# ChristianSteger/HORAYZON

Measured on AMD Instinct MI355X. Metric: grid_cells_per_s (horizon_gridded, 360 azimuths, 3601^2 SRTM-like tile), higher is better.
Workload: dtype f32

## Files before the change

### horayzon_amd/csrc/hz_common.h

```cpp
#pragma once
#include <stdint.h>
#include <hip/hip_runtime.h>

#define HZ_BLOB_MAGIC 0x485a4c42u
#define HZ_BLOB_VERSION 10u
#define HZ_WAVE 64

struct BlobHeader {
    uint32_t magic, version;
    int32_t d0, d1;
    int32_t n_quads, n_tin, n_prims, n_nodes;
    int32_t height, n_top;
    float center[3];
    float pad;
    float lo[3], hi[3];
    uint32_t reserved0[2];
    uint64_t off_verts, off_nodes, off_prims, total_bytes;
    uint64_t off_anc;
    int32_t anc_levels;
    int32_t n_prim_slots;
    uint32_t flags;
    uint32_t n_flipped;
    uint64_t off_bad;
    int32_t bad_nb;
// ... 223 lines not shown
typedef int hz_int2 __attribute__((ext_vector_type(2)));

__device__ __forceinline__ float hz_fma_mix_lo(uint32_t h2, float a, float b) {
    return __builtin_fmaf((float)__builtin_bit_cast(hz_half2, h2).x, a, b);
}
__device__ __forceinline__ float hz_fma_mix_hi(uint32_t h2, float a, float b) {
    return __builtin_fmaf((float)__builtin_bit_cast(hz_half2, h2).y, a, b);
}

__device__ __forceinline__ void hz_node_hits(const NodeRay &n, const RayBox &r, float tfar, const uint4 &q,
                                             bool &h0, bool &h1, bool &h2, bool &h3) {
    const uint32_t px0 = __builtin_amdgcn_perm(HZ_HALF_MAGIC, q.x, r.sel_x), px1 = __builtin_amdgcn_perm(HZ_HALF_MAGIC, q.x, r.sel_x + HZ_SEL_PAIR1);
    const uint32_t py0 = __builtin_amdgcn_perm(HZ_HALF_MAGIC, q.y, r.sel_y), py1 = __builtin_amdgcn_perm(HZ_HALF_MAGIC, q.y, r.sel_y + HZ_SEL_PAIR1);
    const uint32_t pz0 = __builtin_amdgcn_perm(HZ_HALF_MAGIC, q.z, r.sel_z), pz1 = __builtin_amdgcn_perm(HZ_HALF_MAGIC, q.z, r.sel_z + HZ_SEL_PAIR1);
    const uint32_t pz2 = __builtin_amdgcn_perm(HZ_HALF_MAGIC, q.w, r.sel_z), pz3 = __builtin_amdgcn_perm(HZ_HALF_MAGIC, q.w, r.sel_z + HZ_SEL_PAIR1);
    const float nx0 = hz_fma_mix_lo(px0, n.ax, n.bx), fx0 = hz_fma_mix_hi(px0, n.ax, n.bx);
    const float nx1 = hz_fma_mix_lo(px1, n.ax, n.bx), fx1 = hz_fma_mix_hi(px1, n.ax, n.bx);
    const float ny0 = hz_fma_mix_lo(py0, n.ay, n.by), fy0 = hz_fma_mix_hi(py0, n.ay, n.by);
    const float ny1 = hz_fma_mix_lo(py1, n.ay, n.by), fy1 = hz_fma_mix_hi(py1, n.ay, n.by);
    const float cx0 = __builtin_fmaxf(nx0, 0.0f), cx1 = __builtin_fmaxf(nx1, 0.0f);
    const float gx0 = __builtin_fminf(fx0, tfar), gx1 = __builtin_fminf(fx1, tfar);
#define HZ_CHILD(pz, nx, fx, ny, fy, out) do { \
        const float nz_ = hz_fma_mix_lo(pz, n.az, n.bz), fz_ = hz_fma_mix_hi(pz, n.az, n.bz); \
        const float tmin_ = __builtin_fmaxf(__builtin_fmaxf(nx, ny), nz_); \
        const float tmax_ = __builtin_fminf(__builtin_fminf(fx, fy), fz_); \
        out = tmin_ <= tmax_ * 1.000001f; } while (0)
    HZ_CHILD(pz0, cx0, gx0, ny0, fy0, h0);
    HZ_CHILD(pz1, cx1, gx1, ny0, fy0, h1);
    HZ_CHILD(pz2, cx0, gx0, ny1, fy1, h2);
    HZ_CHILD(pz3, cx1, gx1, ny1, fy1, h3);
#undef HZ_CHILD
}

__device__ __forceinline__ void hz_node_hit_masks(const NodeRay &n, const RayBox &r, float tfar, const uint4 &q,
                                                  int &m0, int &m1, int &m2, int &m3) {
    const uint32_t px0 = __builtin_amdgcn_perm(HZ_HALF_MAGIC, q.x, r.sel_x), px1 = __builtin_amdgcn_perm(HZ_HALF_MAGIC, q.x, r.sel_x + HZ_SEL_PAIR1);
    const uint32_t py0 = __builtin_amdgcn_perm(HZ_HALF_MAGIC, q.y, r.sel_y), py1 = __builtin_amdgcn_perm(HZ_HALF_MAGIC, q.y, r.sel_y + HZ_SEL_PAIR1);
    const uint32_t pz0 = __builtin_amdgcn_perm(HZ_HALF_MAGIC, q.z, r.sel_z), pz1 = __builtin_amdgcn_perm(HZ_HALF_MAGIC, q.z, r.sel_z + HZ_SEL_PAIR1);
    const uint32_t pz2 = __builtin_amdgcn_perm(HZ_HALF_MAGIC, q.w, r.sel_z), pz3 = __builtin_amdgcn_perm(HZ_HALF_MAGIC, q.w, r.sel_z + HZ_SEL_PAIR1);
    const float nx0 = hz_fma_mix_lo(px0, n.ax, n.bx), fx0 = hz_fma_mix_hi(px0, n.ax, n.bx);
    const float nx1 = hz_fma_mix_lo(px1, n.ax, n.bx), fx1 = hz_fma_mix_hi(px1, n.ax, n.bx);
    const float ny0 = hz_fma_mix_lo(py0, n.ay, n.by), fy0 = hz_fma_mix_hi(py0, n.ay, n.by);
    const float ny1 = hz_fma_mix_lo(py1, n.ay, n.by), fy1 = hz_fma_mix_hi(py1, n.ay, n.by);
    const float cx0 = __builtin_fmaxf(nx0, 0.0f), cx1 = __builtin_fmaxf(nx1, 0.0f);
    const float gx0 = __builtin_fminf(fx0, tfar), gx1 = __builtin_fminf(fx1, tfar);
#define HZ_CHILD_M(pz, nx, fx, ny, fy, out) do { \
        const float nz_ = hz_fma_mix_lo(pz, n.az, n.bz), fz_ = hz_fma_mix_hi(pz, n.az, n.bz); \
        const float tmin_ = __builtin_fmaxf(__builtin_fmaxf(nx, ny), nz_); \
        const float tmax_ = __builtin_fminf(__builtin_fminf(fx, fy), fz_); \
        out = __float_as_int(__builtin_fmaf(tmax_, -1.000001f, tmin_)) >> 31; \
        asm volatile("" : "+v"(out));      \
        } while (0)
    HZ_CHILD_M(pz0, cx0, gx0, ny0, fy0, m0);
    HZ_CHILD_M(pz1, cx1, gx1, ny0, fy0, m1);
    HZ_CHILD_M(pz2, cx0, gx0, ny1, fy1, m2);
    HZ_CHILD_M(pz3, cx1, gx1, ny1, fy1, m3);
#undef HZ_CHILD_M
}

__device__ __forceinline__ void hz_load_node(const Node *n, float4 &n0, uint4 &n1) {
    asm volatile("global_load_dwordx4 %0, %2, off\n\t"
                 "global_load_dwordx4 %1, %2, off offset:16\n\t"
                 "s_waitcnt vmcnt(0)"
                 : "=&v"(n0), "=&v"(n1)
                 : "v"(n)
                 : "memory");
}

__device__ __forceinline__ void hz_load_node_lds(const float4 *q, float4 &n0, uint4 &n1) {
    const unsigned addr = (unsigned)(size_t)reinterpret_cast<const __attribute__((address_space(3))) char *>(
        (const __attribute__((address_space(3))) float4 *)q);
    asm volatile("ds_read_b128 %0, %2\n\t"
                 "ds_read_b128 %1, %2 offset:16\n\t"
                 "s_waitcnt lgkmcnt(0)"
                 : "=&v"(n0), "=&v"(n1)
                 : "v"(addr)
                 : "memory");
}

__device__ __forceinline__ void hz_load_prim(const Prim *q, float4 &q0, float4 &q1, float4 &q2) {
    asm volatile("global_load_dwordx4 %0, %3, off\n\t"
                 "global_load_dwordx4 %1, %3, off offset:16\n\t"
                 "global_load_dwordx4 %2, %3, off offset:32\n\t"
                 "s_waitcnt vmcnt(0)"
                 : "=&v"(q0), "=&v"(q1), "=&v"(q2)
                 : "v"(q)
                 : "memory");
}

struct TravCounters { unsigned nodes, tris, w_nodes, w_leaves;
};
#endif

#if defined(__HIPCC__)
__host__ __device__
#endif
inline int hz_n_leave(int regroup, int n_entry, int rule, int round) {
    const int cap = rule ? 64 : regroup, share = rule ? regroup : 64;
    const int rel = (share * n_entry + round) >> 6;
    const int cut = cap < rel ? cap : rel;
    return cut > 1 ? cut : 1;
}

#ifdef __HIPCC__
struct LendCounters { unsigned lent, unhelped; };
struct TravState { int node, sp, pf, pm, lq0, lq1; };

__device__ __forceinline__ void hz_trav_reset(TravState &t) {
    t.node = 0; t.sp = 0; t.pf = 0; t.pm = 0; t.lq0 = HZ_EMPTY; t.lq1 = HZ_EMPTY;
}

__device__ __forceinline__ int hz_entry_pack(int pf, int pm) {
    return (int)((unsigned)pf | (((unsigned)pm >> 1) & 3u) | (((unsigned)pm & 8u) << 27));
}
__device__ __forceinline__ void hz_entry_unpack(int e, int &pf, int &pm) {
    pm = (int)((((unsigned)e & 3u) << 1) | (((unsigned)e >> 27) & 8u));
    pf = (int)((unsigned)e & 0xbffffffcu);
}

#define HZ_WAVE_TICK(c, lane_) do { const unsigned long long m_ = __ballot(1); if ((lane_) == __ffsll((long long)m_) - 1) (c)++; } while (0)

template <int TPB, bool COUNT, int QLEN = 2, bool NODELET = false, bool LEVELSTACK = true, bool LEND = false>
__device__ __forceinline__ int hz_trace(const Node *__restrict__ nodes, const Prim *__restrict__ prims,
                                        const float4 *top, int ntop, int *stack, int tid,
                                        float ox, float oy, float oz, float dx, float dy, float dz, float tfar,
                                        float tfar_box, const RayBox &rb, TravState &t, int regroup, int leaf_bias,
                                        TravCounters &cnt, int stack_cap, bool &overflow, LendCounters *lcnt = nullptr,
                                        int regroup_rule = 0) {
    const int lane = tid & 63;
    int node = t.node, sp = t.sp, pf = t.pf, pm = t.pm, lq0 = t.lq0, lq1 = t.lq1;
    const int n_entry = __popcll(__ballot(1));
#define HZ_POP() do { \
        if (LEVELSTACK) { \
            if (pm == 0) { const bool ne = sp > 0; sp = ne ? sp - 1 : 0; const int pv = stack[sp * TPB + tid]; \
                           hz_entry_unpack(ne ? pv : 0, pf, pm); } \
            const int slot_ = __builtin_ctz((unsigned)pm | 16u); \
            node = (pm != 0) ? pf + slot_ : HZ_EMPTY; pm &= pm - 1; \
        } else { \
            node = HZ_STACK_AT(sa + (unsigned)(TPB * 4)); sa -= (unsigned)(TPB * 4); \
        } } while (0)
typedef __attribute__((address_space(3))) int hz_lds_int;
#define HZ_STACK_AT(addr) (*reinterpret_cast<hz_lds_int *>((size_t)(addr)))
#define HZ_SAVE() do { if (!LEVELSTACK) sp = (int)(sa - sa0) / (TPB * 4) + 1; \
                       t.node = node; t.sp = sp; t.pf = pf; t.pm = pm; t.lq0 = lq0; t.lq1 = lq1; } while (0)
    const unsigned sa0 = (unsigned)(size_t)reinterpret_cast<hz_lds_int *>(
                             (__attribute__((address_space(3))) char *)reinterpret_cast<char *>(stack)) + (unsigned)tid * 4u;
    unsigned sa = sa0 + (unsigned)(sp - 1) * (unsigned)(TPB * 4);
    const unsigned sa_cap = sa0 + (unsigned)(stack_cap - 5) * (unsigned)(TPB * 4);
    if (!LEVELSTACK) HZ_STACK_AT(sa0) = HZ_EMPTY;
    unsigned sa_hi = 0u;
    const int n_leave = hz_n_leave(regroup, n_entry, regroup_rule & 1, regroup_rule >> 1);
    bool can_node, can_leaf;
    unsigned long long m_node, m_leaf;
    int n_all;
    auto top_of_iteration = [&]() __attribute__((always_inline)) {
        if (LEVELSTACK) {
            if (node < 0 && lq0 >= 0) { lq0 = node; HZ_POP(); }
            if (node < 0 && lq1 >= 0) { lq1 = node; HZ_POP(); }
        } else {
            hz_int2 t10;
            asm volatile("ds_read2st64_b32 %0, %1 offset1:%2\n\ts_waitcnt lgkmcnt(0)" : "=v"(t10) : "v"(sa), "n"(TPB / 64) : "memory");
            int t0 = t10.y;
            const int t1 = t10.x;
#define HZ_SELM(m, x, y) (((m) & (x)) | (~(m) & (y)))
            int m1 = (node & ~lq0) >> 31;
            asm volatile("" : "+v"(m1));
            lq0 = HZ_SELM(m1, node, lq0); node = HZ_SELM(m1, t0, node); t0 = HZ_SELM(m1, t1, t0); sa -= (unsigned)m1 & (unsigned)(TPB * 4);
            int m2 = (node & ~lq1) >> 31;
            asm volatile("" : "+v"(m2));
            lq1 = HZ_SELM(m2, node, lq1); node = HZ_SELM(m2, t0, node); sa -= (unsigned)m2 & (unsigned)(TPB * 4);
#undef HZ_SELM
        }
        can_node = HZ_IS_NODE(node);
        can_leaf = lq0 < 0;
        m_node = __ballot(can_node); m_leaf = __ballot(can_leaf);
        n_all = __popcll(m_node | m_leaf);
    };
    top_of_iteration();
    while (n_all >= n_leave) {
        const int n_node = __popcll(m_node);
        const int n_leaf = __popcll(m_leaf);
        if (n_node * 16 >= n_leaf * leaf_bias) {
            if (can_node) {
                float4 n0; uint4 n1;
                if (NODELET && node < ntop) hz_load_node_lds(top + 2 * node, n0, n1);
                else hz_load_node(nodes + node, n0, n1);
                if (COUNT) { cnt.nodes++; HZ_WAVE_TICK(cnt.w_nodes, lane); }
                const NodeRay nr = hz_node_ray(rb, n0.x, n0.y, n0.z);
                const int first = __float_as_int(n0.w);
                if (LEVELSTACK) {
                    bool h0, h1, h2, h3;
                    hz_node_hits(nr, rb, tfar_box, n1, h0, h1, h2, h3);
                    const int h = (h0 ? 1 : 0) | (h1 ? 2 : 0) | (h2 ? 4 : 0) | (h3 ? 8 : 0);
                    if (h != 0) {
                        if (pm != 0) { stack[sp * TPB + tid] = hz_entry_pack(pf, pm); sp++; }
                        pf = first; pm = h;
                    }
                    HZ_POP();
                } else {
                    int m0, m1, m2, m3;
                    hz_node_hit_masks(nr, rb, tfar_box, n1, m0, m1, m2, m3);
                    sa_hi = max(sa_hi, sa);
                    sa = min(sa, sa_cap);
                    const unsigned S = (unsigned)(TPB * 4);
                    const int pv = HZ_STACK_AT(sa + S);
                    const unsigned a0 = (unsigned)m0 & S, a1 = (unsigned)m1 & S, a2 = (unsigned)m2 & S, a3 = (unsigned)m3 & S;
                    const unsigned o32 = a3 | a2, o321 = o32 | a1, o3210 = o321 | a0;
#define HZ_SEL(m, x, y) (((m) & (x)) | (~(m) & (y)))
                    int next = HZ_SEL(m3, first + 3, pv);
                    HZ_STACK_AT(sa + 2u * S) = next; sa += a2 & a3;   next = HZ_SEL(m2, first + 2, next);
                    HZ_STACK_AT(sa + 2u * S) = next; sa += a1 & o32;  next = HZ_SEL(m1, first + 1, next);
                    HZ_STACK_AT(sa + 2u * S) = next; sa += a0 & o321; next = HZ_SEL(m0, first, next);
#undef HZ_SEL
                    node = next; sa = sa + o3210 - S;
                }
            }
        } else {
            if (LEND && !LEVELSTACK) {
                static_assert(HZ_EMPTY > 1, "the idle word must be neither a queued link (negative) nor HZ_EMPTY");
                int p_w = 0, lf;
                float rox, roy, roz, rdx, rdy, rdz;
#define HZ_DPP_SEL(d, x) "v_cndmask_b32_dpp %[" d "], %[" x "], %[" x "], vcc quad_perm:[1,0,3,2] row_mask:0xf bank_mask:0xf bound_ctrl:1\n\t"
                asm volatile("s_mov_b64 vcc, %[m]\n\t"
                             "v_cndmask_b32_e32 %[lf], 1, %[lq1], vcc\n\t"
                             HZ_DPP_SEL("rox", "ox") HZ_DPP_SEL("roy", "oy") HZ_DPP_SEL("roz", "oz")
                             HZ_DPP_SEL("rdx", "dx") HZ_DPP_SEL("rdy", "dy") HZ_DPP_SEL("rdz", "dz")
                             "v_mov_b32_dpp %[pw], %[lf] quad_perm:[1,0,3,2] row_mask:0xf bank_mask:0xf\n\t"
                             "v_cndmask_b32_e32 %[lf], %[pw], %[lq0], vcc"
                             : [pw] "+&v"(p_w), [lf] "=&v"(lf), [rox] "=&v"(rox), [roy] "=&v"(roy), [roz] "=&v"(roz),
                               [rdx] "=&v"(rdx), [rdy] "=&v"(rdy), [rdz] "=&v"(rdz)
                             : [m] "s"(m_leaf), [lq0] "v"(lq0), [lq1] "v"(lq1), [ox] "v"(ox), [oy] "v"(oy), [oz] "v"(oz),
                               [dx] "v"(dx), [dy] "v"(dy), [dz] "v"(dz)
                             : "vcc");
#undef HZ_DPP_SEL
// ... 84 lines not shown
```

### horayzon_amd/csrc/hz_horizon.hip

```cpp
#include "hz_search.h"
#include <vector>

namespace hz {

#ifndef HZ_TPB
#define HZ_TPB 256
#endif
#define HZ_WPB (HZ_TPB / 64)
#ifndef HZ_QLEN
#define HZ_QLEN 2
#endif

struct HorizonParams {
    SceneView sv;
    Tables tb;
    const float *vec_norm, *vec_north;
    const uint8_t *mask;
    float *hori;
    int offset_0, offset_1, dim_in_1;
    int row_begin, row_end;
    TileMap tm;
    float dist, hori_fill, ray_org_elev;
    float dist_box, neg_tau;
    int top_nodes, regroup, stack_bytes, leaf_bias, stage_bytes, hit_cache, stack_cap;
    int pre_bytes;
    const unsigned short *near_idx;
    const float *near_r;
    float *scratch_row;
    int verify_near;
    unsigned verify_mask;
    unsigned long long *counters;
    const int *tile_list;
    int n_list;
// ... 20 lines not shown
#ifndef HZ_WG_PER_CU
#define HZ_WG_PER_CU 5
#endif
__global__ __launch_bounds__(HZ_TPB, (COUNT ? 4 : HZ_WG_PER_CU) * (4 / HZ_WPB)) void k_horizon(HorizonParams p_arg) {
    typedef const __attribute__((address_space(4))) HorizonParams *hz_kparams;
    hz_kparams pk = (hz_kparams)__builtin_amdgcn_kernarg_segment_ptr();
#if defined(__HIP_DEVICE_COMPILE__)
#define HZ_LOAD_PARAMS(dst) dst = *pk
#else
#define HZ_LOAD_PARAMS(dst) dst = p_arg
#endif
    HorizonParams p;
    HZ_LOAD_PARAMS(p);
    extern __shared__ __attribute__((aligned(16))) unsigned char smem[];
    int *stack = reinterpret_cast<int *>(smem + p.pre_bytes);
    const float4 *top = reinterpret_cast<const float4 *>(smem + p.pre_bytes + p.stack_bytes);
    const int tid = threadIdx.x;
    const int ntop = p.top_nodes;
    if (NODELET && ntop > 0) {
        float4 *dst = reinterpret_cast<float4 *>(smem + p.pre_bytes + p.stack_bytes);
        const float4 *src = reinterpret_cast<const float4 *>(p.sv.nodes);
        for (int i = tid; i < ntop * 2; i += HZ_TPB) dst[i] = src[i];
        __syncthreads();
    }

    const int wave = __builtin_amdgcn_readfirstlane(tid >> 6);
    const int xcc_own = (int)(__builtin_amdgcn_s_getreg((3 << 11) | 20) & 7u);
    int xcc_off = 0;
    int left_on = 1;
  for (;;) {
    asm volatile("" : "+s"(pk));
    HZ_LOAD_PARAMS(p);
    int tid_b = tid;
    asm volatile("" : "+v"(tid_b));
    const int lane = tid_b & 63;
#define HZ_KEEP(x) asm volatile("" : "+s"(x))
    HZ_KEEP(p.leaf_bias); HZ_KEEP(p.regroup); HZ_KEEP(p.neg_tau); HZ_KEEP(p.sv.cx); HZ_KEEP(p.sv.cy); HZ_KEEP(p.sv.cz);
    HZ_KEEP(p.near_idx); HZ_KEEP(p.near_r);
    if (FLAT && LEFT) { HZ_KEEP(p.sv.nodes); HZ_KEEP(p.sv.prims); }
#undef HZ_KEEP
    int ti = 0, tj = 0;
    int blk = (int)blockIdx.x * HZ_WPB + wave;
    unsigned rec0 = 0u, rec_n = 0u;
    if (LEFT) {
        blk = -1;
        const unsigned groups = (p.left_in_ctl[1] + 63u) / 64u;
        if (p.tile_list) {
            const int b = (int)blockIdx.x * HZ_WPB + wave;
            const int g = b < p.n_list ? p.tile_list[b] : -1;
            if (g >= 0 && (unsigned)g < groups) { blk = g; rec0 = (unsigned)g * 64u; rec_n = min(64u, p.left_in_ctl[1] - (unsigned)g * 64u); }
        } else
        while (xcc_off < 8) {
            const unsigned x = (unsigned)((xcc_own + xcc_off) & 7);
            unsigned q = 0u;
            if (lane == 0) q = atomicAdd(&p.left_in_ctl[8 + x], 1u);
            q = (unsigned)__builtin_amdgcn_readfirstlane((int)q);
            const unsigned g = (((q >> 5) * 8u + x) << 5) | (q & 31u);
            if (g < groups) { blk = (int)g; rec0 = g * 64u; rec_n = min(64u, p.left_in_ctl[1] - g * 64u); break; }
            xcc_off++;
        }
        if (blk < 0) break;
    } else if (p.persist) {
        blk = -1;
        while (xcc_off < 8) {
            const int x = (xcc_own + xcc_off) & 7;
            int q = 0;
            if (lane == 0) q = (int)atomicAdd(&p.queue[x], 1u);
            q = __builtin_amdgcn_readfirstlane(q);
            if (q < p.tm.per_xcd * 4) { blk = (((q >> 2) * 8 + x) << 2) | (q & 3); break; }
            xcc_off++;
        }
        if (blk < 0) break;
    } else if (p.tile_list) blk = (blk < p.n_list) ? p.tile_list[blk] : -1;
// ... 1 lines not shown
        const int b = (int)blockIdx.x, x = b & 7, t = b >> 3, per = 4 / HZ_WPB;
        blk = (((t / per) * 8 + x) * 4) + (t % per) * HZ_WPB + wave;
    }
    blk = __builtin_amdgcn_readfirstlane(blk);
    bool has_tile = blk >= 0 && (LEFT || hz_tile_of_block(p.tm, blk >> 2, &ti, &tj));
    int i = p.row_begin + ti * 16 + ((blk >> 1) & 1) * 8 + (lane >> 3);
    int j = tj * 16 + (blk & 1) * 8 + (lane & 7);
    const unsigned *rec = nullptr;
    if (LEFT) {
        has_tile = (unsigned)lane < rec_n;
        if (has_tile) {
            rec = p.left_rec + ((size_t)p.left_in_base + (size_t)p.left_perm[rec0 + (unsigned)lane]) * HZ_LEFT_WORDS;
            const unsigned c0 = rec[0];
            has_tile = c0 != 0xffffffffu;
            const unsigned di = c0 / (unsigned)p.dim_in_1;
            i = p.row_begin + (int)di; j = (int)(c0 - di * (unsigned)p.dim_in_1);
        }
    }
    const bool in_dom = has_tile && (i < p.row_end) && (j < p.dim_in_1);

    const Tables &t = p.tb;
    const unsigned long long t_start = COUNT ? (unsigned long long)wall_clock64() : 0ull;
    const size_t cell = in_dom ? ((size_t)i * p.dim_in_1 + j) : 0;
    bool done = !in_dom;
    const unsigned cert = in_dom ? (unsigned)(i - p.row_begin) * (unsigned)p.dim_in_1 + (unsigned)j : 0u;
    const bool to_scratch = COUNT && p.scratch_row != nullptr;
    float *const hori0 = to_scratch ? p.scratch_row : p.hori + (size_t)p.row_begin * p.dim_in_1 * (size_t)t.azim_num;
    const unsigned cell_stride = to_scratch ? 0u : 1u;
    Sink out;
    out.hori = COUNT ? hori0 + (size_t)(cert * cell_stride) * (size_t)t.azim_num : hori0 + (size_t)cert * (size_t)t.azim_num;
    out.dist = nullptr; out.dist_hit = 0.0f;
    out.stage = reinterpret_cast<float *>(smem) + tid_b;
    out.stride = HZ_TPB;
    float ox = 0, oy = 0, oz = 0;
    float r01 = 0, r02 = 0, r11 = 0, r12 = 0, r21 = 0, r22 = 0;
    const bool masked = in_dom && p.mask[cell] != 1;
    {
        unsigned long long m = __ballot(masked);
        while (m) {
            const int src = __ffsll((long long)m) - 1;
            m &= m - 1;
            float *row = COUNT ? hori0 + (size_t)((unsigned)__shfl((int)cert, src) * cell_stride) * (size_t)t.azim_num
                               : hori0 + (size_t)__shfl((int)cert, src) * (size_t)t.azim_num;
            for (int k = lane; k < t.azim_num; k += 64) row[k] = p.hori_fill;
        }
    }
    if (in_dom) {
        if (masked) {
            done = true;
        } else {
            const float norm_x = p.vec_norm[3 * cell], norm_y = p.vec_norm[3 * cell + 1], norm_z = p.vec_norm[3 * cell + 2];
            const float north_x = p.vec_north[3 * cell], north_y = p.vec_north[3 * cell + 1], north_z = p.vec_north[3 * cell + 2];
            const float *v = p.sv.verts + 3 * ((size_t)(i + p.offset_0) * p.sv.d1 + (size_t)(j + p.offset_1));
            ox = v[0] + norm_x * p.ray_org_elev;
            oy = v[1] + norm_y * p.ray_org_elev;
            oz = v[2] + norm_z * p.ray_org_elev;
            r01 = north_x; r02 = norm_x;
            r11 = north_y; r12 = norm_y;
            r21 = north_z; r22 = norm_z;
        }
    }
#define HZ_OC(ocx, ocy, ocz) float ocx, ocy, ocz; { float ax_ = ox, ay_ = oy, az_ = oz; \
        asm volatile("" : "+v"(ax_), "+v"(ay_), "+v"(az_)); \
        ocx = ax_ - p.sv.cx; ocy = ay_ - p.sv.cy; ocz = az_ - p.sv.cz; }
    const float tfar = p.dist;

    Search s;
    s.k = 0; s.phase = PH_NEWAZ; s.ind = 0; s.prev = 0; s.pazim = 0; s.count = 0;
    s.lim_up = 0; s.lim_low = 0; s.elev_samp = 0; s.ev = 0;
    unsigned rays = 0, guards = 0, w_adv = 0;
    unsigned refill_hist = 0;
    TravCounters tc; tc.nodes = 0; tc.tris = 0; tc.w_nodes = 0; tc.w_leaves = 0;
    LendCounters lc; lc.lent = 0; lc.unhelped = 0;
    const unsigned cells_cnt = (in_dom && !done && !LEFT) ? 1u : 0u;
    bool ray_active = false, last_hit = false;
    float dx = 0, dy = 0, dz = 1;
    RayBox rb = hz_raybox(0, 0, 0, 0, 0, 1);
    TravState ts; hz_trav_reset(ts);
    int cache = 0;
    bool second = false;
    bool overflow = false;
    unsigned shortened = 0;
    unsigned w_verified = 0, w_violations = 0;
    bool verifying = false, first_result = false, want_v = false;
    float tn = 0.0f;
    bool had_guard = false;
    if (LEFT && !done) {
        s.k = (int)rec[1]; s.phase = (int)(rec[2] & 0xffu); s.ind = (int)rec[3]; s.prev = (int)rec[4]; s.pazim = (int)rec[5]; s.count = (int)rec[6];
        s.lim_up = __uint_as_float(rec[7]); s.lim_low = __uint_as_float(rec[8]); s.elev_samp = __uint_as_float(rec[9]); s.ev = __uint_as_float(rec[10]);
        cache = (int)rec[11];
        last_hit = (rec[2] & 0x100u) != 0u;
        had_guard = (rec[2] & 0x400u) != 0u;
        if (STAGE) { out.stage[0] = __uint_as_float(rec[12]); out.stage[out.stride] = __uint_as_float(rec[13]); out.stage[2 * out.stride] = __uint_as_float(rec[14]); }
        if (rec[2] & 0x200u) {
            const float ec = t.elev_cos[s.ind], es = t.elev_sin[s.ind];
            const float rx = ec * t.azim_sin[s.k], ry = ec * t.azim_cos[s.k], rz = es;
            const float r00 = r11 * r22 - r21 * r12, r10 = r21 * r02 - r01 * r22, r20 = r01 * r12 - r11 * r02;
            dx = (r00 * rx + r01 * ry) + r02 * rz;
            dy = (r10 * rx + r11 * ry) + r12 * rz;
            dz = (r20 * rx + r21 * ry) + r22 * rz;
            HZ_OC(ocx, ocy, ocz)
            rb = hz_raybox(ocx + p.neg_tau * dx, ocy + p.neg_tau * dy, ocz + p.neg_tau * dz, dx, dy, dz);
            hz_trav_reset(ts);
            ray_active = true;
        }
    }

    int left_min = (COUNT || !left_on || __popcll(__ballot(!done)) <= p.left_min + 8) ? 0 : p.left_min;
    while (__ballot(!done) != 0ull) {
        if (!COUNT && left_min > 0 && __popcll(__ballot(!done)) <= left_min) {
            const unsigned long long um = __ballot(!done);
            if (um != 0ull && !(!LEVELSTACK && __ballot(overflow) != 0ull)) {
                const unsigned n = (unsigned)__popcll(um);
                unsigned *const out_rec = p.left_rec + (size_t)p.left_out_base * HZ_LEFT_WORDS;
                unsigned base = 0u;
                if (lane == 0) base = atomicAdd(&p.left_out_ctl[0], n);
                base = (unsigned)__builtin_amdgcn_readfirstlane((int)base);
                if (base + n > p.left_out_cap) {
                    left_on = 0; left_min = 0;
                    if (base + (unsigned)lane < p.left_out_cap) out_rec[(size_t)(base + (unsigned)lane) * HZ_LEFT_WORDS] = 0xffffffffu;
                } else {
                    if (lane == 0) atomicAdd(&p.counters[LEFT ? HZ_CNT_LEFT_AGAIN : HZ_CNT_LEFT_CELLS], (unsigned long long)n);
                    if (!done) {
                        const unsigned rank = (unsigned)__builtin_amdgcn_mbcnt_hi((unsigned)(um >> 32), __builtin_amdgcn_mbcnt_lo((unsigned)um, 0u));
                        const unsigned flags = (unsigned)s.phase | (last_hit ? 0x100u : 0u) | (ray_active ? 0x200u : 0u) | ((guards != 0u || had_guard) ? 0x400u : 0u);
                        hz_left_write(out_rec + (size_t)(base + rank) * HZ_LEFT_WORDS, cert, (unsigned)s.k, flags,
                                      (unsigned)s.ind, (unsigned)s.prev, (unsigned)s.pazim, (unsigned)s.count, s.lim_up, s.lim_low, s.elev_samp, s.ev, (unsigned)cache,
                                      STAGE ? out.stage[0] : 0.0f, STAGE ? out.stage[out.stride] : 0.0f, STAGE ? out.stage[2 * out.stride] : 0.0f);
                        done = true;
                    }
                }
            }
        }

        if (__ballot(!done) == 0ull) break;
        const int n_refill = COUNT ? __popcll(__ballot(!done && !ray_active)) : 0;
        if (COUNT && n_refill > 0 && lane == ((n_refill - 1) >> 3)) refill_hist++;
        if (!done && !ray_active) {
            if (COUNT) HZ_WAVE_TICK(w_adv, lane);
            unsigned cert_r = cert;
            asm volatile("" : "+v"(cert_r));
            out.hori = COUNT ? hori0 + (size_t)(cert_r * cell_stride) * (size_t)t.azim_num : hori0 + (size_t)cert_r * (size_t)t.azim_num;
#define HZ_RAY_SETUP(GO) \
                const float rx = ec * asn, ry = ec * acs, rz = es; \
                float nx_ = r01, ny_ = r11, nz_ = r21;         \
                asm volatile("" : "+v"(nx_), "+v"(ny_), "+v"(nz_)); \
                const float r00 = ny_ * r22 - nz_ * r12;       \
                const float r10 = nz_ * r02 - nx_ * r22; \
                const float r20 = nx_ * r12 - ny_ * r02; \
                dx = (r00 * rx + r01 * ry) + r02 * rz; \
                dy = (r10 * rx + r11 * ry) + r12 * rz; \
                dz = (r20 * rx + r21 * ry) + r22 * rz; \
                    tn = (s.ind >= near_i) ? near_rad : p.neg_tau;     \
                if (COUNT && (GO) && tn > 0.0f) shortened++; \
                if (COUNT) want_v = (GO) && p.verify_near && tn > 0.0f && (((rays + cert) & p.verify_mask) == 0u); \
                HZ_OC(ocx, ocy, ocz) \
                rb = hz_raybox(ocx + tn * dx, ocy + tn * dy, ocz + tn * dz, dx, dy, dz); \
                hz_trav_reset(ts); \
                 \
                second = p.hit_cache && (cache != 0) && (s.ind <= s.pazim) && (s.k > 0); \
                if (second) { \
                    ts.node = cache; \
                     \
                    if (!LEVELSTACK) { ts.sp = 1; stack[HZ_TPB + tid] = 0; second = false; } \
                }
            if (FLAT) {
                float ec = 0.0f, es = 0.0f, asn = 0.0f, acs = 0.0f, near_rad = 0.0f;
                int near_i = 0x7fffffff;
                const bool go = advance_guess_flat<STAGE>(s, last_hit, t, out, guards,
                    [&](int kc) {
                        asn = t.azim_sin[kc]; acs = t.azim_cos[kc];
                        if (p.near_idx != nullptr) {
                            near_i = (int)p.near_idx[(size_t)cert_r * (size_t)t.azim_num + kc];
                            near_rad = p.near_r[cert_r];
                        }
                    },
                    [&](int ind) { ec = t.elev_cos[ind]; es = t.elev_sin[ind]; });
                HZ_RAY_SETUP(go)
                ray_active = go;
                done = !go;
                rays += go ? 1u : 0u;
            } else
            if (advance<ALG, STAGE>(s, last_hit, t, out, guards)) {
                const float ec = t.elev_cos[s.ind], es = t.elev_sin[s.ind];
                const float asn = t.azim_sin[s.k], acs = t.azim_cos[s.k];
                int near_i = 0x7fffffff;
                float near_rad = 0.0f;
                if (p.near_idx != nullptr) {
                    near_i = (int)p.near_idx[(size_t)cert_r * (size_t)t.azim_num + s.k];
                    near_rad = p.near_r[cert_r];
                }
                HZ_RAY_SETUP(true)
                ray_active = true;
                rays++;
            } else {
                done = true;
            }
#undef HZ_RAY_SETUP
        }
        bool start_v = false, viol = false;
        if (COUNT && n_refill > 0) {
            const int n_enter = __popcll(__ballot(ray_active));
            if (n_enter > 0 && lane == 8 + ((n_enter - 1) >> 3)) refill_hist++;
        }
        if (ray_active) {
            int r;
            r = hz_trace<HZ_TPB, COUNT, HZ_QLEN, NODELET, LEVELSTACK, LEND>(p.sv.nodes, p.sv.prims, top, ntop, stack, tid, ox, oy, oz,
                                                 dx, dy, dz, tfar, p.dist_box, rb, ts, p.regroup & 0xff, p.leaf_bias, tc, p.stack_cap, overflow, &lc, p.regroup >> 8);
            if (r == 0 && second) {
                second = false; hz_trav_reset(ts);
            } else if (COUNT && want_v && r != 2) {
                want_v = false; verifying = true; first_result = (r == 1); start_v = true;
                HZ_OC(ocx, ocy, ocz)
                rb = hz_raybox(ocx + p.neg_tau * dx, ocy + p.neg_tau * dy, ocz + p.neg_tau * dz, dx, dy, dz);
                hz_trav_reset(ts);
            } else if (r != 2) {
                if (COUNT && verifying) { viol = ((r == 1) != first_result); verifying = false; }
                ray_active = false; last_hit = (r == 1);
                if (r == 1) cache = p.sv.anc[HZ_LEAF_ID(ts.lq0)];
            }
        }
        if (COUNT) {
            w_verified += (unsigned)__popcll(__ballot(start_v));
            w_violations += (unsigned)__popcll(__ballot(viol));
        }
    }
    unsigned long long r = rays, g = guards, nc = tc.nodes, tcn = tc.tris, cc = cells_cnt;
    unsigned long long wn = tc.w_nodes, wl = tc.w_leaves, wa = w_adv;
    unsigned long long ln = lc.lent, un = lc.unhelped;
    for (int off = 32; off > 0; off >>= 1) {
        r += __shfl_xor(r, off); g += __shfl_xor(g, off); cc += __shfl_xor(cc, off);
        if (COUNT) {
            nc += __shfl_xor(nc, off); tcn += __shfl_xor(tcn, off);
            wn += __shfl_xor(wn, off); wl += __shfl_xor(wl, off); wa += __shfl_xor(wa, off);
            if (LEND) { ln += __shfl_xor(ln, off); un += __shfl_xor(un, off); }
        }
    }
    const bool wave_overflowed = !LEVELSTACK && __ballot(overflow) != 0ull;
    if (wave_overflowed) {
        if (lane == 0) {
            const unsigned long long slot = atomicAdd(&p.counters[LEFT ? HZ_CNT_LEFT_OVERFLOW : HZ_CNT_OVERFLOW], 1ull);
            if (slot < (unsigned long long)HZ_REDO_CAP) p.redo_list[(LEFT ? HZ_REDO_CAP : 0) + (int)slot] = blk;
        }
    } else {
    const int guard_cells = __popcll(__ballot(guards != 0u && !(LEFT && had_guard)));
    if (lane == 0) {
        if (r) atomicAdd(&p.counters[HZ_CNT_RAYS], r);
        if (g) { atomicAdd(&p.counters[HZ_CNT_GUARDS], g); atomicAdd(&p.counters[HZ_CNT_GUARD_CELLS], (unsigned long long)guard_cells); }
        if (cc) atomicAdd(&p.counters[HZ_CNT_CELLS], cc);
        if (COUNT) {
            atomicAdd(&p.counters[HZ_CNT_NODES], nc); atomicAdd(&p.counters[HZ_CNT_TRIS], tcn);
            atomicAdd(&p.counters[HZ_CNT_WAVE_NODE], wn); atomicAdd(&p.counters[HZ_CNT_WAVE_LEAF], wl); atomicAdd(&p.counters[HZ_CNT_WAVE_REFILL], wa);
            if (LEND) { atomicAdd(&p.counters[HZ_CNT_LENT], ln); atomicAdd(&p.counters[HZ_CNT_UNHELPED], un); }
        }
    }
    if (COUNT && lane < 16 && refill_hist != 0u) atomicAdd(&p.counters[HZ_CNT_REFILL + lane], (unsigned long long)refill_hist);
    if (COUNT) {
        if (lane == 0) {
            const unsigned xcc = __builtin_amdgcn_s_getreg((3 << 11) | 20) & 7u;
            atomicMax(&p.counters[HZ_CNT_XCD_END + xcc], (unsigned long long)wall_clock64());
            atomicMax(&p.counters[HZ_CNT_START], ~t_start);
        }
    }
    if (COUNT) {
        unsigned long long sh = shortened;
        for (int off = 32; off > 0; off >>= 1) sh += __shfl_xor(sh, off);
        if (lane == 0) {
            if (sh) atomicAdd(&p.counters[HZ_CNT_SHORTENED], sh);
            if (w_violations) atomicAdd(&p.counters[HZ_CNT_VIOLATIONS], (unsigned long long)w_violations);
            if (w_verified) atomicAdd(&p.counters[HZ_CNT_VERIFIED], (unsigned long long)w_verified);
        }
    }
    }
    if (!p.persist) break;
  }
}

std::atomic<int> g_leaf_lend{1};
std::atomic<int> g_flat_refill{1};
std::atomic<int> g_regroup_rule{1};
std::atomic<int> g_regroup_round{HZ_REGROUP_ROUND};

static long long resident_workgroups(const void *func, size_t lds) {
    struct Key { const void *f; size_t lds; int dev; long long n; };
    static std::mutex mu;
    static std::vector<Key> cache;
    int dev = 0;
    if (hipGetDevice(&dev) != hipSuccess) { (void)hipGetLastError(); return 0; }
    std::lock_guard<std::mutex> lock(mu);
    for (const Key &k : cache) if (k.f == func && k.lds == lds && k.dev == dev) return k.n;
    int per_cu = 0;
    hipDeviceProp_t prop;
    long long n = 0;
    if (hipOccupancyMaxActiveBlocksPerMultiprocessor(&per_cu, func, HZ_TPB, lds) == hipSuccess && per_cu > 0 &&
        hipGetDeviceProperties(&prop, dev) == hipSuccess && prop.multiProcessorCount > 0)
        n = (long long)per_cu * prop.multiProcessorCount;
    else (void)hipGetLastError();
    cache.push_back(Key{func, lds, dev, n});
    return n;
}

template <int ALG, bool COUNT, bool STAGE, bool NODELET, bool LEVELSTACK, bool LEND = false, bool FLAT = false>
static int launch_one(const HorizonParams &p_in, int grid, size_t lds, int persist_grid, hipStream_t st) {
    const void *func = reinterpret_cast<const void *>(k_horizon<ALG, COUNT, STAGE, NODELET, LEVELSTACK, false, LEND, FLAT>);
    HZ_HIP(hipFuncSetAttribute(func, hipFuncAttributeMaxDynamicSharedMemorySize, (int)lds));
    HorizonParams p = p_in;
    if (p.persist) {
        const long long resident = persist_grid > 0 ? (long long)persist_grid : resident_workgroups(func, lds);
// ... 512 lines not shown
```

### horayzon_amd/csrc/hz_search.h

```cpp
#pragma once
#include "hz_internal.h"

namespace hz {

enum { ALG_DISCRETE = 0, ALG_BINARY = 1, ALG_GUESS = 2 };
enum { PH_NEWAZ = 0, PH_BIN = 1, PH_UP = 2, PH_DOWN = 3, PH_EMIT = 4 };

struct Tables {
    const float *azim_sin, *azim_cos, *elev_ang, *elev_sin, *elev_cos;
    const int *mid_idx;
    int azim_num, elev_num;
    float hori_acc, low, up;
    double step;
};

struct Search {
    int k, phase, ind, prev, pazim, count;
    float lim_up, lim_low, elev_samp;
    float ev;
};

__device__ __forceinline__ int ind_of(const Tables &t, float elev_samp) {
    return (int)__builtin_roundf((float)((double)(elev_samp - t.low) / t.step));
}
// ... 85 lines not shown
            }
            if (guard) guards++;
            if (ALG == ALG_DISCRETE) {
                s.ev = half_sum(t.elev_ang[s.prev], t.elev_ang[s.ind]); s.phase = PH_EMIT;
                s.pazim = s.prev;
                continue;
            }
            if (s.count > 1) {
                s.ind = mid_index(t, s.prev, s.ind, &s.ev);
                s.pazim = s.ind; s.phase = PH_EMIT;
                continue;
            }
            s.ind = min(s.pazim + 5, top);
            s.prev = s.ind;
            s.ind = max(s.ind - 10, 0);
            s.phase = PH_DOWN;
            return true;
        }
        {
            const bool guard = (!hit) && (s.ind == 0);
            if (!hit && !guard) {
                s.prev = s.ind;
                s.ind = max(s.ind - 10, 0);
                return true;
            }
            if (guard) guards++;
            s.ind = mid_index(t, s.prev, s.ind, &s.ev);
            s.pazim = s.ind; s.phase = PH_EMIT;
            continue;
        }
    }
}

#define HZ_HIDE(m) asm volatile("" : "+v"(m))
#define HZ_BSEL(m, x, y) (((m) & (x)) | (~(m) & (y)))
template <bool STAGE, class FK, class FI>
__device__ __forceinline__ bool advance_guess_flat(Search &s, bool hit, const Tables &t, Sink &out, unsigned &guards,
                                                   FK &&issue_k, FI &&issue_ind) {
    const int top = t.elev_num - 1;
    int m_flat = (int)((unsigned)s.phase << 30) >> 31;
    HZ_HIDE(m_flat);
    if (__ballot(m_flat == 0) != 0ull) {
        if (m_flat == 0) (void)advance<ALG_GUESS, STAGE>(s, hit, t, out, guards);
    }
    int m_down = (int)((unsigned)s.phase << 31) >> 31;
    int m_hit = hit ? -1 : 0;
    int m_end = (s.ind == (top & ~m_down)) ? -1 : 0;
    int m_many = (1 - s.count) >> 31;
    HZ_HIDE(m_down); HZ_HIDE(m_hit); HZ_HIDE(m_end); HZ_HIDE(m_many);
    const int m_fwd = (m_hit ^ m_down) & m_flat;
    const int m_step = m_fwd & ~m_end;
    const int m_turn = m_flat & ~(m_step | m_down | m_many);
    const int m_fin = m_flat & ~(m_step | m_turn);
    guards += (unsigned)(m_fwd & m_end & 1);
    const int st_ind = min(max(s.ind + 10 - (20 & m_down), 0), top);
    const int tu_prev = min(s.pazim + 5, top), tu_ind = max(tu_prev - 10, 0);
    const int lo = min(s.prev, s.ind), hi = max(s.prev, s.ind);
    const int2 pair = reinterpret_cast<const int2 *>(t.mid_idx)[min(max(lo, 0), top)];
    int m_gen = (hi - lo != 10) ? m_fin : 0;
    HZ_HIDE(m_gen);
    const int k_new = s.k - m_fin;
    issue_k(min(k_new, t.azim_num - 1));
    int mid = pair.x, evb = pair.y;
    if (__ballot(m_gen != 0) != 0ull) {
        if (m_gen != 0) {
            mid = ind_of(t, half_sum(t.elev_ang[s.prev], t.elev_ang[s.ind]));
            evb = __float_as_int(t.elev_ang[mid]);
        }
    }
    const int fi_prev = max(mid - 5, 0), fi_ind = min(fi_prev + 10, top);
    const int ind_new = HZ_BSEL(m_step, st_ind, HZ_BSEL(m_turn, tu_ind, HZ_BSEL(m_fin, fi_ind, s.ind)));
    issue_ind(ind_new);
    const int k_emit = s.k;
    s.prev = HZ_BSEL(m_step, s.ind, HZ_BSEL(m_turn, tu_prev, HZ_BSEL(m_fin, fi_prev, s.prev)));
    s.ind = ind_new;
    s.count = HZ_BSEL(m_fin, 1, s.count + (m_step & ~m_down & 1));
    s.phase += m_turn & 1;
    s.phase -= m_fin & m_down & 1;
    s.pazim = HZ_BSEL(m_fin, mid, s.pazim);
    s.ev = __int_as_float(HZ_BSEL(m_fin, evb, __float_as_int(s.ev)));
    s.k = k_new;
    if (m_fin != 0) emit<STAGE>(out, t, k_emit, __int_as_float(evb));
    return s.k < t.azim_num;
}
#undef HZ_BSEL
#undef HZ_HIDE

}
```

Measured before the change: 10.93 million.

## Add lean FLAT path with slim search state and absolute LDS stack address

For the FLAT kernel variant, the search state shrinks to SearchLean: the bisection limits move into LDS staging slots and the unused ev/elev_samp fields are dropped. The traversal stack pointer is now kept as an absolute LDS byte address, and the regroup parameters are pre-packed into one scalar. The box test takes tfar as an SGPR operand through inline asm, and the sel_x1/sel_y1 selectors are hoisted out of the loop. The aim is to lower VGPR pressure and per-iteration integer work to raise occupancy, at the cost of extra LDS traffic and more complicated suspend/resume record handling.

```diff
diff --git a/horayzon_amd/csrc/hz_common.h b/horayzon_amd/csrc/hz_common.h
--- a/horayzon_amd/csrc/hz_common.h
+++ b/horayzon_amd/csrc/hz_common.h
@@ -279,10 +279,16 @@
 #undef HZ_CHILD
 }
 
-__device__ __forceinline__ void hz_node_hit_masks(const NodeRay &n, const RayBox &r, float tfar, const uint4 &q,
-                                                  int &m0, int &m1, int &m2, int &m3) {
-    const uint32_t px0 = __builtin_amdgcn_perm(HZ_HALF_MAGIC, q.x, r.sel_x), px1 = __builtin_amdgcn_perm(HZ_HALF_MAGIC, q.x, r.sel_x + HZ_SEL_PAIR1);
-    const uint32_t py0 = __builtin_amdgcn_perm(HZ_HALF_MAGIC, q.y, r.sel_y), py1 = __builtin_amdgcn_perm(HZ_HALF_MAGIC, q.y, r.sel_y + HZ_SEL_PAIR1);
+__device__ __forceinline__ float hz_min_uniform(float a, float uniform_b) {
+    float r;
+    asm("v_min_f32_e32 %0, %2, %1" : "=v"(r) : "v"(a), "s"(uniform_b));
+    return r;
+}
+template <bool LEAN>
+__device__ __forceinline__ void hz_node_hit_masks_t(const NodeRay &n, const RayBox &r, uint32_t sel_x1, uint32_t sel_y1, float tfar, const uint4 &q,
+                                                    int &m0, int &m1, int &m2, int &m3) {
+    const uint32_t px0 = __builtin_amdgcn_perm(HZ_HALF_MAGIC, q.x, r.sel_x), px1 = __builtin_amdgcn_perm(HZ_HALF_MAGIC, q.x, sel_x1);
+    const uint32_t py0 = __builtin_amdgcn_perm(HZ_HALF_MAGIC, q.y, r.sel_y), py1 = __builtin_amdgcn_perm(HZ_HALF_MAGIC, q.y, sel_y1);
     const uint32_t pz0 = __builtin_amdgcn_perm(HZ_HALF_MAGIC, q.z, r.sel_z), pz1 = __builtin_amdgcn_perm(HZ_HALF_MAGIC, q.z, r.sel_z + HZ_SEL_PAIR1);
     const uint32_t pz2 = __builtin_amdgcn_perm(HZ_HALF_MAGIC, q.w, r.sel_z), pz3 = __builtin_amdgcn_perm(HZ_HALF_MAGIC, q.w, r.sel_z + HZ_SEL_PAIR1);
     const float nx0 = hz_fma_mix_lo(px0, n.ax, n.bx), fx0 = hz_fma_mix_hi(px0, n.ax, n.bx);
@@ -290,7 +296,7 @@
     const float ny0 = hz_fma_mix_lo(py0, n.ay, n.by), fy0 = hz_fma_mix_hi(py0, n.ay, n.by);
     const float ny1 = hz_fma_mix_lo(py1, n.ay, n.by), fy1 = hz_fma_mix_hi(py1, n.ay, n.by);
     const float cx0 = __builtin_fmaxf(nx0, 0.0f), cx1 = __builtin_fmaxf(nx1, 0.0f);
-    const float gx0 = __builtin_fminf(fx0, tfar), gx1 = __builtin_fminf(fx1, tfar);
+    const float gx0 = LEAN ? hz_min_uniform(fx0, tfar) : __builtin_fminf(fx0, tfar), gx1 = LEAN ? hz_min_uniform(fx1, tfar) : __builtin_fminf(fx1, tfar);
 #define HZ_CHILD_M(pz, nx, fx, ny, fy, out) do { \
         const float nz_ = hz_fma_mix_lo(pz, n.az, n.bz), fz_ = hz_fma_mix_hi(pz, n.az, n.bz); \
         const float tmin_ = __builtin_fmaxf(__builtin_fmaxf(nx, ny), nz_); \
@@ -304,6 +310,10 @@
     HZ_CHILD_M(pz3, cx1, gx1, ny1, fy1, m3);
 #undef HZ_CHILD_M
 }
+__device__ __forceinline__ void hz_node_hit_masks(const NodeRay &n, const RayBox &r, float tfar, const uint4 &q,
+                                                  int &m0, int &m1, int &m2, int &m3) {
+    hz_node_hit_masks_t<false>(n, r, r.sel_x + HZ_SEL_PAIR1, r.sel_y + HZ_SEL_PAIR1, tfar, q, m0, m1, m2, m3);
+}
 
 __device__ __forceinline__ void hz_load_node(const Node *n, float4 &n0, uint4 &n1) {
     asm volatile("global_load_dwordx4 %0, %2, off\n\t"
@@ -348,6 +358,20 @@
     const int cut = cap < rel ? cap : rel;
     return cut > 1 ? cut : 1;
 }
+#if defined(__HIPCC__)
+__host__ __device__
+#endif
+inline int hz_n_leave_pack(int regroup, int rule, int round) {
+    return (rule ? 64 : regroup) | ((rule ? regroup : 64) << 8) | (round << 16);
+}
+#if defined(__HIPCC__)
+__host__ __device__
+#endif
+inline int hz_n_leave_packed(int pack, int n_entry) {
+    const int cap = pack & 0xff, rel = (((pack >> 8) & 0xff) * n_entry + (pack >> 16)) >> 6;
+    const int cut = cap < rel ? cap : rel;
+    return cut > 1 ? cut : 1;
+}
 
 #ifdef __HIPCC__
 struct LendCounters { unsigned lent, unhelped; };
@@ -356,6 +380,15 @@
 __device__ __forceinline__ void hz_trav_reset(TravState &t) {
     t.node = 0; t.sp = 0; t.pf = 0; t.pm = 0; t.lq0 = HZ_EMPTY; t.lq1 = HZ_EMPTY;
 }
+__device__ __forceinline__ void hz_lds_store(unsigned lds_byte_address, int v) {
+    *reinterpret_cast<__attribute__((address_space(3))) int *>((size_t)lds_byte_address) = v;
+}
+template <int TPB>
+__device__ __forceinline__ int hz_trav_sa(const int *stack, int tid, int sp) {
+    const unsigned sa0 = (unsigned)(size_t)reinterpret_cast<__attribute__((address_space(3))) int *>(
+                             (__attribute__((address_space(3))) char *)reinterpret_cast<char *>(const_cast<int *>(stack))) + (unsigned)tid * 4u;
+    return (int)(sa0 + (unsigned)(sp - 1) * (unsigned)(TPB * 4));
+}
 
 __device__ __forceinline__ int hz_entry_pack(int pf, int pm) {
     return (int)((unsigned)pf | (((unsigned)pm >> 1) & 3u) | (((unsigned)pm & 8u) << 27));
@@ -367,7 +400,7 @@
 
 #define HZ_WAVE_TICK(c, lane_) do { const unsigned long long m_ = __ballot(1); if ((lane_) == __ffsll((long long)m_) - 1) (c)++; } while (0)
 
-template <int TPB, bool COUNT, int QLEN = 2, bool NODELET = false, bool LEVELSTACK = true, bool LEND = false>
+template <int TPB, bool COUNT, int QLEN = 2, bool NODELET = false, bool LEVELSTACK = true, bool LEND = false, bool LEAN = false>
 __device__ __forceinline__ int hz_trace(const Node *__restrict__ nodes, const Prim *__restrict__ prims,
                                         const float4 *top, int ntop, int *stack, int tid,
                                         float ox, float oy, float oz, float dx, float dy, float dz, float tfar,
@@ -388,15 +421,19 @@
         } } while (0)
 typedef __attribute__((address_space(3))) int hz_lds_int;
 #define HZ_STACK_AT(addr) (*reinterpret_cast<hz_lds_int *>((size_t)(addr)))
-#define HZ_SAVE() do { if (!LEVELSTACK) sp = (int)(sa - sa0) / (TPB * 4) + 1; \
+#define HZ_SAVE() do { if (!LEVELSTACK) sp = LEAN ? (int)sa : (int)(sa - sa0) / (TPB * 4) + 1; \
                        t.node = node; t.sp = sp; t.pf = pf; t.pm = pm; t.lq0 = lq0; t.lq1 = lq1; } while (0)
     const unsigned sa0 = (unsigned)(size_t)reinterpret_cast<hz_lds_int *>(
                              (__attribute__((address_space(3))) char *)reinterpret_cast<char *>(stack)) + (unsigned)tid * 4u;
-    unsigned sa = sa0 + (unsigned)(sp - 1) * (unsigned)(TPB * 4);
+    static_assert(!LEAN || !LEVELSTACK, "LEAN is a form of the fast stack");
+    unsigned sa = LEAN ? (unsigned)sp : sa0 + (unsigned)(sp - 1) * (unsigned)(TPB * 4);
     const unsigned sa_cap = sa0 + (unsigned)(stack_cap - 5) * (unsigned)(TPB * 4);
-    if (!LEVELSTACK) HZ_STACK_AT(sa0) = HZ_EMPTY;
+    if (!LEVELSTACK && !LEAN) HZ_STACK_AT(sa0) = HZ_EMPTY;
     unsigned sa_hi = 0u;
-    const int n_leave = hz_n_leave(regroup, n_entry, regroup_rule & 1, regroup_rule >> 1);
+    const int n_leave = LEAN ? hz_n_leave_packed(regroup, n_entry)
+                             : hz_n_leave(regroup, n_entry, regroup_rule & 1, regroup_rule >> 1);
+    uint32_t sel_x1 = rb.sel_x + HZ_SEL_PAIR1, sel_y1 = rb.sel_y + HZ_SEL_PAIR1;
+    if (LEAN) asm volatile("" : "+v"(sel_x1), "+v"(sel_y1));
     bool can_node, can_leaf;
     unsigned long long m_node, m_leaf;
     int n_all;
@@ -431,6 +468,7 @@
             if (can_node) {
                 float4 n0; uint4 n1;
                 if (NODELET && node < ntop) hz_load_node_lds(top + 2 * node, n0, n1);
+                else if (LEAN) hz_load_node(nodes + (unsigned)node, n0, n1);
                 else hz_load_node(nodes + node, n0, n1);
                 if (COUNT) { cnt.nodes++; HZ_WAVE_TICK(cnt.w_nodes, lane); }
                 const NodeRay nr = hz_node_ray(rb, n0.x, n0.y, n0.z);
@@ -446,7 +484,8 @@
                     HZ_POP();
                 } else {
                     int m0, m1, m2, m3;
-                    hz_node_hit_masks(nr, rb, tfar_box, n1, m0, m1, m2, m3);
+                    if (LEAN) hz_node_hit_masks_t<true>(nr, rb, sel_x1, sel_y1, tfar_box, n1, m0, m1, m2, m3);
+                    else hz_node_hit_masks(nr, rb, tfar_box, n1, m0, m1, m2, m3);
                     sa_hi = max(sa_hi, sa);
                     sa = min(sa, sa_cap);
                     const unsigned S = (unsigned)(TPB * 4);
diff --git a/horayzon_amd/csrc/hz_horizon.hip b/horayzon_amd/csrc/hz_horizon.hip
--- a/horayzon_amd/csrc/hz_horizon.hip
+++ b/horayzon_amd/csrc/hz_horizon.hip
@@ -1,4 +1,5 @@
 #include "hz_search.h"
+#include <type_traits>
 #include <vector>
 
 namespace hz {
@@ -85,13 +86,21 @@
     asm volatile("" : "+s"(pk));
     HZ_LOAD_PARAMS(p);
     int tid_b = tid;
+    if (FLAT) {
+        int zero = 0;
+        asm volatile("" : "+v"(zero));
+        tid_b = (wave << 6) | (int)__builtin_amdgcn_mbcnt_hi(~0u, __builtin_amdgcn_mbcnt_lo(~0u, (unsigned)zero));
+    }
     asm volatile("" : "+v"(tid_b));
     const int lane = tid_b & 63;
 #define HZ_KEEP(x) asm volatile("" : "+s"(x))
+    if (FLAT) p.regroup = hz_n_leave_pack(p.regroup & 0xff, (p.regroup >> 8) & 1, p.regroup >> 9);
     HZ_KEEP(p.leaf_bias); HZ_KEEP(p.regroup); HZ_KEEP(p.neg_tau); HZ_KEEP(p.sv.cx); HZ_KEEP(p.sv.cy); HZ_KEEP(p.sv.cz);
     HZ_KEEP(p.near_idx); HZ_KEEP(p.near_r);
     if (FLAT && LEFT) { HZ_KEEP(p.sv.nodes); HZ_KEEP(p.sv.prims); }
 #undef HZ_KEEP
+    typedef const __attribute__((address_space(1))) unsigned short *hz_gl_u16;
+    typedef const __attribute__((address_space(1))) float *hz_gl_f32;
     int ti = 0, tj = 0;
     int blk = (int)blockIdx.x * HZ_WPB + wave;
     unsigned rec0 = 0u, rec_n = 0u;
@@ -159,6 +168,9 @@
     out.dist = nullptr; out.dist_hit = 0.0f;
     out.stage = reinterpret_cast<float *>(smem) + tid_b;
     out.stride = HZ_TPB;
+    float *const lim = out.stage + (STAGE ? 2 : 0) * HZ_TPB;
+    static_assert(!FLAT || !LEVELSTACK, "the flat refill is built for the fast stack");
+    if (FLAT) stack[tid_b] = HZ_EMPTY;
     float ox = 0, oy = 0, oz = 0;
     float r01 = 0, r02 = 0, r11 = 0, r12 = 0, r21 = 0, r22 = 0;
     const bool masked = in_dom && p.mask[cell] != 1;
@@ -192,9 +204,9 @@
         ocx = ax_ - p.sv.cx; ocy = ay_ - p.sv.cy; ocz = az_ - p.sv.cz; }
     const float tfar = p.dist;
 
-    Search s;
+    typename std::conditional<FLAT, SearchLean, Search>::type s;
     s.k = 0; s.phase = PH_NEWAZ; s.ind = 0; s.prev = 0; s.pazim = 0; s.count = 0;
-    s.lim_up = 0; s.lim_low = 0; s.elev_samp = 0; s.ev = 0;
+    if constexpr (!FLAT) { s.lim_up = 0; s.lim_low = 0; s.elev_samp = 0; s.ev = 0; }
     unsigned rays = 0, guards = 0, w_adv = 0;
     unsigned refill_hist = 0;
     TravCounters tc; tc.nodes = 0; tc.tris = 0; tc.w_nodes = 0; tc.w_leaves = 0;
@@ -203,7 +215,9 @@
     bool ray_active = false, last_hit = false;
     float dx = 0, dy = 0, dz = 1;
     RayBox rb = hz_raybox(0, 0, 0, 0, 0, 1);
-    TravState ts; hz_trav_reset(ts);
+#define HZ_TS_RESET(SP) do { hz_trav_reset(ts); if (FLAT) { int tid_r = tid_b; asm volatile("" : "+v"(tid_r)); \
+                             ts.sp = hz_trav_sa<HZ_TPB>(stack, tid_r, (SP)); } else ts.sp = (SP); } while (0)
+    TravState ts; HZ_TS_RESET(0);
     int cache = 0;
     bool second = false;
     bool overflow = false;
@@ -214,11 +228,12 @@
     bool had_guard = false;
     if (LEFT && !done) {
         s.k = (int)rec[1]; s.phase = (int)(rec[2] & 0xffu); s.ind = (int)rec[3]; s.prev = (int)rec[4]; s.pazim = (int)rec[5]; s.count = (int)rec[6];
-        s.lim_up = __uint_as_float(rec[7]); s.lim_low = __uint_as_float(rec[8]); s.elev_samp = __uint_as_float(rec[9]); s.ev = __uint_as_float(rec[10]);
+        if constexpr (!FLAT) { s.lim_up = __uint_as_float(rec[7]); s.lim_low = __uint_as_float(rec[8]); s.elev_samp = __uint_as_float(rec[9]); s.ev = __uint_as_float(rec[10]); }
         cache = (int)rec[11];
         last_hit = (rec[2] & 0x100u) != 0u;
         had_guard = (rec[2] & 0x400u) != 0u;
         if (STAGE) { out.stage[0] = __uint_as_float(rec[12]); out.stage[out.stride] = __uint_as_float(rec[13]); out.stage[2 * out.stride] = __uint_as_float(rec[14]); }
+        if (FLAT && s.phase == PH_BIN) { lim[0] = __uint_as_float(rec[7]); lim[HZ_TPB] = __uint_as_float(rec[8]); }
         if (rec[2] & 0x200u) {
             const float ec = t.elev_cos[s.ind], es = t.elev_sin[s.ind];
             const float rx = ec * t.azim_sin[s.k], ry = ec * t.azim_cos[s.k], rz = es;
@@ -228,7 +243,7 @@
             dz = (r20 * rx + r21 * ry) + r22 * rz;
             HZ_OC(ocx, ocy, ocz)
             rb = hz_raybox(ocx + p.neg_tau * dx, ocy + p.neg_tau * dy, ocz + p.neg_tau * dz, dx, dy, dz);
-            hz_trav_reset(ts);
+            HZ_TS_RESET(0);
             ray_active = true;
         }
     }
@@ -251,8 +266,11 @@
                     if (!done) {
                         const unsigned rank = (unsigned)__builtin_amdgcn_mbcnt_hi((unsigned)(um >> 32), __builtin_amdgcn_mbcnt_lo((unsigned)um, 0u));
                         const unsigned flags = (unsigned)s.phase | (last_hit ? 0x100u : 0u) | (ray_active ? 0x200u : 0u) | ((guards != 0u || had_guard) ? 0x400u : 0u);
+                        float w7 = 0.0f, w8 = 0.0f, w9 = 0.0f, w10 = 0.0f;
+                        if constexpr (FLAT) { if (s.phase == PH_BIN) { w7 = lim[0]; w8 = lim[HZ_TPB]; } }
+                        else { w7 = s.lim_up; w8 = s.lim_low; w9 = s.elev_samp; w10 = s.ev; }
                         hz_left_write(out_rec + (size_t)(base + rank) * HZ_LEFT_WORDS, cert, (unsigned)s.k, flags,
-                                      (unsigned)s.ind, (unsigned)s.prev, (unsigned)s.pazim, (unsigned)s.count, s.lim_up, s.lim_low, s.elev_samp, s.ev, (unsigned)cache,
+                                      (unsigned)s.ind, (unsigned)s.prev, (unsigned)s.pazim, (unsigned)s.count, w7, w8, w9, w10, (unsigned)cache,
                                       STAGE ? out.stage[0] : 0.0f, STAGE ? out.stage[out.stride] : 0.0f, STAGE ? out.stage[2 * out.stride] : 0.0f);
                         done = true;
                     }
@@ -283,23 +301,24 @@
                 if (COUNT) want_v = (GO) && p.verify_near && tn > 0.0f && (((rays + cert) & p.verify_mask) == 0u); \
                 HZ_OC(ocx, ocy, ocz) \
                 rb = hz_raybox(ocx + tn * dx, ocy + tn * dy, ocz + tn * dz, dx, dy, dz); \
-                hz_trav_reset(ts); \
+                HZ_TS_RESET(0); \
                  \
                 second = p.hit_cache && (cache != 0) && (s.ind <= s.pazim) && (s.k > 0); \
                 if (second) { \
                     ts.node = cache; \
                      \
-                    if (!LEVELSTACK) { ts.sp = 1; stack[HZ_TPB + tid] = 0; second = false; } \
+                    if (FLAT) { ts.sp += HZ_TPB * 4; hz_lds_store((unsigned)ts.sp + (unsigned)(HZ_TPB * 4), 0); second = false; }       \
+                    else if (!LEVELSTACK) { ts.sp = 1; stack[HZ_TPB + tid] = 0; second = false; } \
                 }
-            if (FLAT) {
+            if constexpr (FLAT) {
                 float ec = 0.0f, es = 0.0f, asn = 0.0f, acs = 0.0f, near_rad = 0.0f;
                 int near_i = 0x7fffffff;
-                const bool go = advance_guess_flat<STAGE>(s, last_hit, t, out, guards,
+                const bool go = advance_guess_flat<STAGE>(s, last_hit, t, out, guards, lim, HZ_TPB,
                     [&](int kc) {
                         asn = t.azim_sin[kc]; acs = t.azim_cos[kc];
                         if (p.near_idx != nullptr) {
-                            near_i = (int)p.near_idx[(size_t)cert_r * (size_t)t.azim_num + kc];
-                            near_rad = p.near_r[cert_r];
+                            near_i = (int)((hz_gl_u16)p.near_idx)[(size_t)cert_r * (size_t)t.azim_num + kc];
+                            near_rad = ((hz_gl_f32)p.near_r)[cert_r];
                         }
                     },
                     [&](int ind) { ec = t.elev_cos[ind]; es = t.elev_sin[ind]; });
@@ -332,15 +351,15 @@
         }
         if (ray_active) {
             int r;
-            r = hz_trace<HZ_TPB, COUNT, HZ_QLEN, NODELET, LEVELSTACK, LEND>(p.sv.nodes, p.sv.prims, top, ntop, stack, tid, ox, oy, oz,
-                                                 dx, dy, dz, tfar, p.dist_box, rb, ts, p.regroup & 0xff, p.leaf_bias, tc, p.stack_cap, overflow, &lc, p.regroup >> 8);
+            r = hz_trace<HZ_TPB, COUNT, HZ_QLEN, NODELET, LEVELSTACK, LEND, FLAT>(p.sv.nodes, p.sv.prims, top, ntop, stack, FLAT ? tid_b : tid, ox, oy, oz,
+                                                 dx, dy, dz, tfar, p.dist_box, rb, ts, FLAT ? p.regroup : (p.regroup & 0xff), p.leaf_bias, tc, p.stack_cap, overflow, &lc, p.regroup >> 8);
             if (r == 0 && second) {
-                second = false; hz_trav_reset(ts);
+                second = false; HZ_TS_RESET(0);
             } else if (COUNT && want_v && r != 2) {
                 want_v = false; verifying = true; first_result = (r == 1); start_v = true;
                 HZ_OC(ocx, ocy, ocz)
                 rb = hz_raybox(ocx + p.neg_tau * dx, ocy + p.neg_tau * dy, ocz + p.neg_tau * dz, dx, dy, dz);
-                hz_trav_reset(ts);
+                HZ_TS_RESET(0);
             } else if (r != 2) {
                 if (COUNT && verifying) { viol = ((r == 1) != first_result); verifying = false; }
                 ray_active = false; last_hit = (r == 1);
@@ -401,6 +420,7 @@
     }
     if (!p.persist) break;
   }
+#undef HZ_TS_RESET
 }
 
 std::atomic<int> g_leaf_lend{1};
diff --git a/horayzon_amd/csrc/hz_search.h b/horayzon_amd/csrc/hz_search.h
--- a/horayzon_amd/csrc/hz_search.h
+++ b/horayzon_amd/csrc/hz_search.h
@@ -141,16 +141,52 @@
     }
 }
 
+struct SearchLean {
+    int k, phase, ind, prev, pazim, count;
+};
+
+template <bool STAGE>
+__device__ __forceinline__ bool advance_az0_lean(SearchLean &s, bool hit, const Tables &t, Sink &out, float *lim, int lim_stride) {
+    const int top = t.elev_num - 1;
+    if (s.phase == PH_NEWAZ && s.k >= t.azim_num) return false;
+    if (s.phase == PH_BIN || s.k == 0) {
+        float lim_up = t.up, lim_low = t.low;
+        if (s.phase == PH_BIN) {
+            const float e0 = t.elev_ang[s.ind];
+            lim_up = lim[0]; lim_low = lim[lim_stride];
+            if (hit) lim_low = e0; else lim_up = e0;
+        }
+        const float elev_samp = half_sum(lim_up, lim_low);
+        s.ind = ind_of(t, elev_samp);
+        s.phase = PH_BIN;
+        const float e = t.elev_ang[s.ind];
+        if (__builtin_fmaxf(lim_up - e, e - lim_low) > t.hori_acc) {
+            lim[0] = lim_up; lim[lim_stride] = lim_low;
+            return true;
+        }
+        s.pazim = s.ind;
+        emit<STAGE>(out, t, s.k, elev_samp);
+        s.k++; s.phase = PH_NEWAZ;
+        if (s.k >= t.azim_num) return false;
+    }
+    s.ind = max(s.pazim - 5, 0);
+    s.prev = s.ind;
+    s.ind = min(s.ind + 10, top);
+    s.count = 1;
+    s.phase = PH_UP;
+    return true;
+}
+
 #define HZ_HIDE(m) asm volatile("" : "+v"(m))
 #define HZ_BSEL(m, x, y) (((m) & (x)) | (~(m) & (y)))
 template <bool STAGE, class FK, class FI>
-__device__ __forceinline__ bool advance_guess_flat(Search &s, bool hit, const Tables &t, Sink &out, unsigned &guards,
-                                                   FK &&issue_k, FI &&issue_ind) {
+__device__ __forceinline__ bool advance_guess_flat(SearchLean &s, bool hit, const Tables &t, Sink &out, unsigned &guards,
+                                                   float *lim, int lim_stride, FK &&issue_k, FI &&issue_ind) {
     const int top = t.elev_num - 1;
     int m_flat = (int)((unsigned)s.phase << 30) >> 31;
     HZ_HIDE(m_flat);
     if (__ballot(m_flat == 0) != 0ull) {
-        if (m_flat == 0) (void)advance<ALG_GUESS, STAGE>(s, hit, t, out, guards);
+        if (m_flat == 0) (void)advance_az0_lean<STAGE>(s, hit, t, out, lim, lim_stride);
     }
     int m_down = (int)((unsigned)s.phase << 31) >> 31;
     int m_hit = hit ? -1 : 0;
@@ -187,7 +223,6 @@
     s.phase += m_turn & 1;
     s.phase -= m_fin & m_down & 1;
     s.pazim = HZ_BSEL(m_fin, mid, s.pazim);
-    s.ev = __int_as_float(HZ_BSEL(m_fin, evb, __float_as_int(s.ev)));
     s.k = k_new;
     if (m_fin != 0) emit<STAGE>(out, t, k_emit, __int_as_float(evb));
     return s.k < t.azim_num;
```

Measured after the change: 11.10 million (median of 6 runs). +1.6%, better.
